# zhangzhousuper/Radish_PT

Measured on AMD Instinct MI355X. Metric: Mrays/s, higher is better.
Workload: dtype f32

## Files before the change

### radish_pt_amd/csrc/device/kernels_wave.h

```cpp
#pragma once
#include "kernels_pt.h"
#include "wg_trace.h"
#include "ray_cull.h"

namespace rd {

constexpr int kWfLitCap = 8192;
constexpr int kWfLitShadow = 0x40000000;
constexpr int kMaxWaveDepth = 32;

struct alignas(128) WaveCounter {
    int v;
    int pad[31];
};
#ifndef RD_WF_TICKET_SHARDS
#define RD_WF_TICKET_SHARDS 8
#endif
constexpr int kTicketShards = RD_WF_TICKET_SHARDS;
struct WaveCounters {
    WaveCounter rayCount[kMaxWaveDepth + 2];
    WaveCounter shadowCount[kMaxWaveDepth + 2];
    WaveCounter litCount[kMaxWaveDepth + 2];
    WaveCounter litShadowCount[kMaxWaveDepth + 2];
    WaveCounter traceHead[kMaxWaveDepth + 2];
    WaveCounter shadeHead[kMaxWaveDepth + 2][4];
    WaveCounter traceTicket[kMaxWaveDepth + 2][kTicketShards];
    WaveCounter shadeTicket[kMaxWaveDepth + 2][kTicketShards];
};

struct WaveWorkspace {
    float4 *ro[2];
    float4 *rd[2];
    float4 *thr[2];
    float4 *prevPos[2];
    float4 *accD;
    float4 *accI;
    float4 *nee[2];
    float4 *sht[2];
    uint2 *rng[2];
    int4 *hit;
    int *rayq[2];
    int *shadowq;
    int *litq[2];
    int litCap;
    int *treeOvf;
    int treeOvfDepth;
#ifdef RD_WF_STAMPS
    unsigned long long *stamps;
    int stampWaves;
    int stampStages;
#endif
    WaveCounters *ctr;
};

constexpr unsigned kWfNeeNone = 2u;
RD_DEV float wfNeeTag(int home, unsigned kind) { return __uint_as_float(((unsigned)home << 2) | kind); }
RD_DEV void wfAddNee(const WaveWorkspace &w, float4 n) {
    const unsigned tag = __float_as_uint(n.w), kind = tag & 3u;
    if (kind == kWfNeeNone) return;
    float4 *acc = (kind == 0u ? w.accD : w.accI) + (tag >> 2);
    const float4 a = *acc;
    *acc = make_float4(a.x + n.x, a.y + n.y, a.z + n.z, 0.f);
}

RD_DEV Ray wfSlotRay(const WaveWorkspace &w, int set, int p, bool shadow, float &limit) {
    if (shadow) {
        const float4 x = w.prevPos[set][p], y = w.sht[set][p];
        return shadowRay(mk3(x.x, x.y, x.z), mk3(y.x, y.y, y.z), limit);
    }
    const float4 o = w.ro[set][p], d = w.rd[set][p];
    limit = 3.402823466e+38f;
    return Ray{mk3(o.x, o.y, o.z), mk3(d.x, d.y, d.z)};
}

struct WaveSlotPath {
    const WaveWorkspace &w;
    const int rs, p;
    const int wr, q;
    int home;
    const bool delta;
    bool nullNee = false;
    RD_DEV v3 throughput() {
        const float4 t = w.thr[rs][p];
        home = __float_as_int(t.w);
        return mk3(t.x, t.y, t.z);
    }
// ... 335 lines not shown
                    if (busy && cur >= 0) {
                        pairStep<COUNT>(s.pairs, stk, lane, ovf, rs, tmax, ord, cur, sp, pending, ws);
                        busy = pending < 0 && (cur >= 0 || sp.sp > 0);
                    }
                } while (__popcll(__ballot(busy)) >= (minWalk > 1 ? minWalk : 1));
                alive = alive && (pending >= 0 || cur >= 0 || sp.sp > 0);
            }
        } else
        {
            bool walking = alive && pending < 0;
            const int nStart = __popcll(__ballot(walking));
#if RD_WF_COOP_LONE
            if (nStart == 1) {
                const int L = __ffsll((long long)__ballot(walking)) - 1;
                CoopResult cr = coopWalk(readlanePtr(nodes, L), readlaneI(node, L), end, readlaneRay(rs, L), readlaneF(tmax, L), RD_COOP_WINDOWS);
                if (int(threadIdx.x & 63u) == L) {
                    node = cr.node;
                    pending = cr.pending;
                    if (COUNT) ws.nodes += cr.visited;
                    alive = (node != end) || pending >= 0;
                }
            } else
#endif
            if (nStart > 0) {
                const int minWalk = (nStart * (RD_LEAF_DEN - RD_LEAF_NUM) + RD_LEAF_DEN - 1) / RD_LEAF_DEN;
                do {
                    if (walking) {
                        if (COUNT) ws.nodes++;
                        float4 lo = nodes[node].lo_prim;
                        float4 hi = nodes[node].hi_next;
                        float boundDist;
                        bool boundHit = aabbFast(lo, hi, rs, boundDist);
                        if (boundHit && boundDist < tmax) {
                            pending = __float_as_int(lo.w);
                            node++;
                        } else {
                            node = __float_as_int(hi.w);
                        }
                        walking = pending < 0 && node != END;
                        alive = (node != END) || pending >= 0;
                    }
                } while (__popcll(__ballot(walking)) >= (minWalk > 1 ? minWalk : 1));
            }
        }
        if (alive && pending >= 0) {
            TriVerts t = loadTri(s.tris, pending);
            float dist;
            v2 bary;
            if (COUNT) ws.tris++;
            bool hit = intersectTriangle(rs, t.a, t.b, t.c, bary, dist);
            if (hit && dist < tmax) {
                if (isShadow) {
                    occluded = true;
                    node = END;
                    cur = kPairNone;
                    sp = PairStack{0, 0};
                } else {
                    hitPrim = pending;
                    tmax = dist;
                    hitBary = bary;
                }
            }
            pending = -1;
            alive = PAIRS ? (cur >= 0 || sp.sp > 0) : (node != END);
        }
        const unsigned long long doneM = __ballot(!alive && p >= 0);
        if (doneM != 0ull && __popcll(doneM) * 64 >= (__popcll(doneM) + __popcll(__ballot(alive))) * RD_WF_FINISH_MIN)
        if (!alive && p >= 0) {
            if (isShadow) {
                if (!occluded) wfAddNee(w, w.nee[set][p]);
            } else {
                bool hit = hitPrim != -1;
                if (hit) nHits++;
                w.hit[p] = make_int4(hitPrim, __float_as_int(hit ? hitBary.x : 0.f), __float_as_int(hit ? hitBary.y : 0.f),
                                     hit ? int(s.primClass[hitPrim]) : 0);
            }
            p = -1;
        }
    }
    RD_WF_STAMP(2);
    if (COUNT) flushCounters(s.counters, nClosest, nAny, nHits, ws);
}

constexpr int kSortChunks = 16;
constexpr int kSortPacket = 64 * kSortChunks;
#ifndef RD_WF_SHADE_WAVES
#define RD_WF_SHADE_WAVES 1
#endif
#ifndef RD_WF_CULL_LAST
#define RD_WF_CULL_LAST 1
#endif
#ifndef RD_WF_SKIP_NULL_NEE
#define RD_WF_SKIP_NULL_NEE 1
#endif
__global__ __launch_bounds__(256, RD_WF_SHADE_WAVES) void k_wf_shade(DScene s, WaveWorkspace w, int k, int maxDepth, int sorted,
                                                                     const float4 *__restrict__ emitBox, int walkAll) {
    __shared__ int sSorted[4][kSortPacket];
    WaveCounters *c = w.ctr;
    const bool cullLast = RD_WF_CULL_LAST && !walkAll && k + 1 == maxDepth && !hasEnvMap(s);
    const bool skipNull = RD_WF_SKIP_NULL_NEE && !walkAll;
    float4 boxLo = make_float4(0.f, 0.f, 0.f, 0.f), boxHi = boxLo;
    if (cullLast) {
        boxLo = emitBox[0];
        boxHi = emitBox[1];
    }
    const int wg = workgroupTicket(c->shadeTicket[k]);
    const int lane = int(threadIdx.x & 63u);
    int *mySorted = sSorted[threadIdx.x >> 6];
    {
        const int q = 0;
        const int n = c->rayCount[k].v;
        const int *hitq = w.rayq[k & 1];
        int pendShadows = 0, pendRays = 0;
        int packet = kShadePacket;
        if (sorted) {
            const int perWave = n / (2 * gridWaves());
            packet = ((perWave + kShadePacket - 1) / kShadePacket) * kShadePacket;
            packet = packet < kShadePacket ? kShadePacket : (packet > kSortPacket ? kSortPacket : packet);
        }
        int packetEnd = 0;
        for (int base = logicalWave(wg) * packet, sub = 0, fresh = 1;;) {
            if (sub == packet) {
                base = wavePull(&c->shadeHead[k][q].v, packet);
                sub = 0;
                fresh = 1;
            }
            if (base + sub >= n) break;
            if (sorted && fresh) {
                fresh = 0;
                packetEnd = (n - base) < packet ? (n - base) : packet;
                int pp[kSortChunks], cls[kSortChunks];
#pragma unroll
                for (int j = 0; j < kSortChunks; j++) {
                    const int i = base + j * 64 + lane;
                    pp[j] = (j * 64 + lane < packetEnd) ? hitq[i] : -1;
                    if (pp[j] <= -2) pp[j] = -2 - pp[j];
                }
#pragma unroll
                for (int j = 0; j < kSortChunks; j++) {
                    cls[j] = (pp[j] >= 0) ? w.hit[pp[j]].w : 0;
                }
                int at = 0;
#pragma unroll
                for (int qq = 0; qq < 4; qq++) {
#pragma unroll
                    for (int j = 0; j < kSortChunks; j++) {
                        const bool in = (j * 64 + lane < packetEnd) && cls[j] == qq;
                        const unsigned long long m = __ballot(in);
                        if (in) mySorted[at + __popcll(m & laneMaskLt())] = pp[j];
                        at += __popcll(m);
                    }
                }
                __builtin_amdgcn_wave_barrier();
            }
            int item = base + sub + lane;
            const int subNow = sub;
            sub += 64;
            bool active = sorted ? (subNow + lane < packetEnd) : (item < n);
            bool emitShadow = false, emitRay = false, litShadow = false, litRay = false, rayFirst = false;
            int p = -1;
            const int q = base + subNow + lane;
            if (active) {
                p = sorted ? mySorted[subNow + lane] : hitq[item];
                if (p <= -2) p = -2 - p;
                active = p >= 0;
            }
// ... 89 lines not shown
```

### radish_pt_amd/csrc/radish_hip.hip

```cpp
#include "radish_hip.h"

#include <hip/hip_runtime.h>
#include <dlfcn.h>

#include <algorithm>
#include <cfloat>
#include <climits>
#include <cmath>
#include <cstdarg>
#include <cstdio>
#include <cstring>
#include <mutex>
#include <string>
#include <type_traits>
#include <utility>
#include <vector>

#include "device/kernels_pt.h"
#include "device/kernels_restir.h"
#include "device/kernels_wave.h"
#include "device/kernels_persist.h"
#include "device/kernels_walk.h"
#include "device/kernels_gbuffer.h"
#include "device/kernels_display.h"
// ... 482 lines not shown
            pend[c0 + nb] = pend[b] + 1;
            pend[c0 + (nb ^ 1)] = pend[b];
            if (pend[b] + 1 > depth) depth = pend[b] + 1;
        }
    }
    for (int box = 0; box < S; box++) {
        const int b = canon[box];
        const float *q = d->boundingBoxes + 6 * (size_t)box;
        tree[b].lo_prim = make_float4(q[0], q[1], q[2], asFloat(w3[b]));
        tree[b].hi_next = make_float4(q[3], q[4], q[5], asFloat(bits[b]));
    }
    pairs.assign((size_t)(S - 1) / 2 + 1, PairRec{});
    auto childW = [&](int b) { return w3[b] >= 0 ? w3[b] : ~((~w3[b] - 1) / 2); };
    for (int b = 0; b < S; b++) {
        if (w3[b] >= 0) continue;
        const int c0 = ~w3[b], q = (c0 - 1) / 2;
        const float4 l0 = tree[c0].lo_prim, h0 = tree[c0].hi_next, l1 = tree[c0 + 1].lo_prim, h1 = tree[c0 + 1].hi_next;
        pairs[q].lo0_w0 = make_float4(l0.x, l0.y, l0.z, asFloat(childW(c0)));
        pairs[q].hi0_bits = make_float4(h0.x, h0.y, h0.z, asFloat(bits[b]));
        pairs[q].lo1_w1 = make_float4(l1.x, l1.y, l1.z, asFloat(childW(c0 + 1)));
        pairs[q].hi1_pad = make_float4(h1.x, h1.y, h1.z, asFloat(0));
    }
    return true;
}

struct HostCamera {
    int32_t resx, resy;
    float position[3], rotation[3], view[3], up[3], right[3];
    float fov[2], pixelLength[2];
    float rotationMatInv[9];
    float viewProjection[16];
    float lensRadius, focalDist, tanFovY;
};
static_assert(sizeof(HostCamera) == 196, "Camera layout");

DCamera toDeviceCamera(const void *camera196) {
    HostCamera h;
    memcpy(&h, camera196, sizeof(h));
    DCamera d;
    d.resx = h.resx;
    d.resy = h.resy;
    d.position = {h.position[0], h.position[1], h.position[2]};
    d.view = {h.view[0], h.view[1], h.view[2]};
    d.up = {h.up[0], h.up[1], h.up[2]};
    d.right = {h.right[0], h.right[1], h.right[2]};
    d.rotationMatInv.c0 = {h.rotationMatInv[0], h.rotationMatInv[1], h.rotationMatInv[2]};
    d.rotationMatInv.c1 = {h.rotationMatInv[3], h.rotationMatInv[4], h.rotationMatInv[5]};
    d.rotationMatInv.c2 = {h.rotationMatInv[6], h.rotationMatInv[7], h.rotationMatInv[8]};
    d.lensRadius = h.lensRadius;
    d.focalDist = h.focalDist;
    d.tanFovY = tanf(h.fov[1] * 0.01745329251994329576923690768489f);
    return d;
}

PixelMap makePixelMap(const rdh_ctx *c) {
    PixelMap pm;
    pm.W = c->cam.resx;
    pm.H = c->cam.resy;
    pm.tile = c->tile;
    pm.tilesX = (pm.W + pm.tile - 1) / pm.tile;
    int tilesY = (pm.H + pm.tile - 1) / pm.tile;
    pm.numTiles = pm.tilesX * tilesY;
    pm.rank = c->rank;
    pm.world = c->world;
    pm.tilesPerRank = (pm.numTiles + pm.world - 1) / pm.world;
    pm.packed = (c->world > 1 || c->forcePacked) ? 1 : 0;
    int bpe = pm.tile / 8;
    pm.numBlocks = pm.tilesPerRank * bpe * bpe;
    return pm;
}

constexpr int kPairMinNodes = 0;
bool usePairs(const rdh_ctx *c, uint32_t flags) {
    if (!c->scene.ds.pairs || (flags & RDH_PT_NO_PAIRS)) return false;
    if (flags & RDH_PT_PAIRS) return true;
    if (c->pairMode >= 0) return c->pairMode != 0;
    return c->scene.ds.bvhSize >= kPairMinNodes;
}

bool usePackets(uint32_t flags) {
    static const int env = getenv("RADISH_PACKETS") ? atoi(getenv("RADISH_PACKETS")) : 1;
    return env != 0 && !(flags & RDH_PT_NO_PACKETS);
}

unsigned gridFor(const PixelMap &pm) {
    unsigned work = (unsigned)(pm.numBlocks + 3) / 4;
    return ((work + 7u) / 8u) * 8u;
}

unsigned gridBlocks(const PixelMap &pm) { return (((unsigned)pm.numBlocks + 7u) / 8u) * 8u; }

int settleTree(rdh_ctx *c) {
    if (!c->scene.treePending) return RDH_OK;
    HIP_TRY(c, hipEventSynchronize(c->evTree));
    c->scene.treePending = false;
    if (c->scene.treeRefit) {
        c->scene.treeRefit = false;
        if (!c->scene.ds.pairs) return RDH_OK;
        const int4 lo = c->hTreeHdr.as<int4>()[1], hi = c->hTreeHdr.as<int4>()[2];
        c->scene.ds.rootLo = make_float4(__builtin_bit_cast(float, lo.x), __builtin_bit_cast(float, lo.y), __builtin_bit_cast(float, lo.z), c->scene.ds.rootLo.w);
        c->scene.ds.rootHi = make_float4(__builtin_bit_cast(float, hi.x), __builtin_bit_cast(float, hi.y), __builtin_bit_cast(float, hi.z), c->scene.ds.rootHi.w);
        return RDH_OK;
    }
    const int4 *hdr = c->hTreeHdr.as<int4>(), h0 = hdr[0], lo = hdr[1], hi = hdr[2];
    if (h0.y != 0) {
        c->scene.haveScene = false;
        return fail(c, RDH_ERR_STATE, "device BVH build failed (error bits %d); the scene must be uploaded again", h0.y);
    }
    constexpr int kMaxPairDepth = 2048;
    const PairRec *pairs = c->scene.updPairs ? c->scene.updPairs : c->scene.ds.pairs;
    if (h0.x <= kMaxPairDepth) {
        c->scene.ds.pairs = pairs;
        c->scene.ds.treeDepth = h0.x;
        c->scene.ds.rootLo = make_float4(__builtin_bit_cast(float, lo.x), __builtin_bit_cast(float, lo.y), __builtin_bit_cast(float, lo.z),
                                   __builtin_bit_cast(float, lo.w));
        c->scene.ds.rootHi = make_float4(__builtin_bit_cast(float, hi.x), __builtin_bit_cast(float, hi.y), __builtin_bit_cast(float, hi.z),
                                   __builtin_bit_cast(float, hi.w));
    } else {
        c->scene.ds.pairs = nullptr;
        c->scene.ds.treeDepth = 0;
    }
    return RDH_OK;
}

int settleLights(rdh_ctx *c) {
    if (!c->scene.lightsPending) return RDH_OK;
    HIP_TRY(c, hipEventSynchronize(c->evLights));
    c->scene.lightsPending = false;
    c->scene.ds.sumLightPowerInv = c->hLightSums.as<float>()[1];
    return RDH_OK;
}

int requireReady(rdh_ctx *c) {
    if (!c) return RDH_ERR_ARGS;
    if (c->scene.haveScene) {
        int rc = settleTree(c);
        if (rc) return rc;
        if ((rc = settleLights(c))) return rc;
    }
    if (!c->scene.haveScene) return fail(c, RDH_ERR_NO_SCENE, "no scene uploaded (rdh_scene_upload)");
    if (!c->haveCamera) return fail(c, RDH_ERR_NO_SCENE, "no camera set (rdh_set_camera)");
    return RDH_OK;
}

constexpr size_t kProfilePairs = 8192;

long profBegin(rdh_ctx *c, uint32_t flags) {
    if (!(flags & RDH_PT_PROFILE) || c->profUsed >= kProfilePairs) return -1;
    if (c->profEvents.size() < 2 * (c->profUsed + 1)) {
        hipEvent_t a = nullptr, b = nullptr;
        if (newEvent(c, &a, true) || newEvent(c, &b, true)) return -1;
        c->profEvents.push_back(a);
        c->profEvents.push_back(b);
    }
    long i = (long)c->profUsed++;
    hipEventRecord(c->profEvents[2 * i], c->stream);
    return i;
}
void profEnd(rdh_ctx *c, long i) {
    if (i >= 0) hipEventRecord(c->profEvents[2 * i + 1], c->stream);
}

constexpr unsigned kPersistentGrid = 256u * 8u;

template <typename T>
int wfAlloc(rdh_ctx *c, T **out, size_t count) {
    void *p = nullptr;
    HIP_TRY(c, hipMalloc(&p, std::max<size_t>(count * sizeof(T), 16)));
    c->wfAllocs.push_back(p);
    *out = static_cast<T *>(p);
    return RDH_OK;
}

int wavefrontEnsureSlots(rdh_ctx *c, long long slots) {
    if (c->wfCapacity >= slots) return RDH_OK;
    for (void *p : c->wfAllocs) hipFree(p);
    c->wfAllocs.clear();
    c->wfCapacity = 0;
    const size_t n0 = (size_t)slots, n1 = (size_t)((slots / 64 + 1) / 2) * 64;
    for (int h = 0; h < kWfParts; h++) {
        WaveWorkspace &w = c->wf[h];
        const size_t n = h == 0 ? n0 : n1;
        int rc = RDH_OK;
        for (int set = 0; set < 2 && rc == RDH_OK; set++) {
            if ((rc = wfAlloc(c, &w.ro[set], n)) || (rc = wfAlloc(c, &w.rd[set], n)) || (rc = wfAlloc(c, &w.thr[set], n)) ||
                (rc = wfAlloc(c, &w.prevPos[set], n)) || (rc = wfAlloc(c, &w.nee[set], n)) || (rc = wfAlloc(c, &w.sht[set], n)) ||
                (rc = wfAlloc(c, &w.rng[set], n)))
                return rc;
        }
        if ((rc = wfAlloc(c, &w.accD, n)) || (rc = wfAlloc(c, &w.accI, n)) ||
            (rc = wfAlloc(c, &w.hit, n)) || (rc = wfAlloc(c, &w.rayq[0], n)) || (rc = wfAlloc(c, &w.rayq[1], n)) ||
            (rc = wfAlloc(c, &w.shadowq, n)) || (rc = wfAlloc(c, &w.ctr, 1)) || (rc = wfAlloc(c, &w.litq[0], (size_t)kWfLitCap)) ||
            (rc = wfAlloc(c, &w.litq[1], (size_t)kWfLitCap)))
            return rc;
        w.litCap = 0;
    }
    if (!c->evWfFork) {
        int rc;
        if ((rc = newEvent(c, &c->evWfFork)) || (rc = newEvent(c, &c->evWfJoin))) return rc;
        HIP_TRY(c, hipStreamCreateWithFlags(&c->wfStream, hipStreamNonBlocking));
        if ((rc = newEvent(c, &c->evWfJoin3))) return rc;
    }
    c->wfCapacity = slots;
    return RDH_OK;
}
int wavefrontEnsure(rdh_ctx *c, const PixelMap &pm, int samples) {
    return wavefrontEnsureSlots(c, (long long)pm.numBlocks * 64 * samples);
}

struct WfLaunch {
    bool count, sort, walkAll, tree;
    unsigned traceGrid, shadeGrid;
    int parts;
};
int wavefrontPrepare(rdh_ctx *c, int maxDepth, uint32_t flags, int parts, WfLaunch &L) {
    if (maxDepth > kMaxWaveDepth) return fail(c, RDH_ERR_ARGS, "maxDepth %d exceeds %d", maxDepth, kMaxWaveDepth);
    const bool count = (flags & RDH_PT_COUNT) != 0, sort = (flags & RDH_PT_SORT_MATERIAL) != 0;
    const bool walkAll = count || (flags & RDH_PT_WALK_ALL) != 0 || c->scene.lightListPartial;
    const bool tree = usePairs(c, flags);
    unsigned traceRes = 0, shadeRes = 0;
    int rq = RDH_OK;
    withBools([&](auto cnt, auto pr) { rq = residentGrid(c, k_wf_trace<cnt.value, pr.value>, 256, &traceRes); }, count, tree);
    if (rq || (rq = residentGrid(c, k_wf_shade, 256, &shadeRes))) return rq;
    if (tree && !count) {
        int cus = 0;
        if (int rc = cuCount(c, &cus)) return rc;
        traceRes = std::min(traceRes, (unsigned)cus * (unsigned)RD_WF_PAIR_MAX_WAVES);
    }
    const unsigned traceGrid = sharedGrid(c, std::min(traceRes, kPersistentGrid), kUnbounded);
    const unsigned shadeGrid = sharedGrid(c, std::min(shadeRes, kPersistentGrid), kUnbounded);
    const int ovfDepth = c->scene.ds.treeDepth + 1;
    const size_t ovfNeed = (size_t)traceGrid * 4 * 64 * (size_t)ovfDepth * 2;
    if (tree && parts > 1 && (size_t)parts * ovfNeed * sizeof(int) > kWfStripBudget) parts = 1;
    if (tree) {
        for (int h = 0; h < parts; h++) {
            if (int rc = grow(c, c->wfTreeOvf[h], ovfNeed, ovfNeed * sizeof(int), Busy::Device)) return rc;
            c->wf[h].treeOvf = c->wfTreeOvf[h].as<int>();
            c->wf[h].treeOvfDepth = ovfDepth;
        }
    }
#ifdef RD_WF_STAMPS
    {
        const size_t stamps = (size_t)(maxDepth + 1) * traceGrid * 4 * kWfStampKinds + (size_t)(maxDepth + 1);
        if (int rc = grow(c, c->wfStamps, stamps, stamps * sizeof(unsigned long long), Busy::Device)) return rc;
        HIP_TRY(c, hipMemsetAsync(c->wfStamps.p, 0, stamps * sizeof(unsigned long long), c->stream));
        for (int h = 0; h < kWfParts; h++) {
            c->wf[h].stamps = h == 0 ? c->wfStamps.as<unsigned long long>() : nullptr;
            c->wf[h].stampWaves = (int)(traceGrid * 4);
            c->wf[h].stampStages = maxDepth + 1;
        }
        c->wfStampStages = maxDepth + 1;
        c->wfStampWaves = (int)(traceGrid * 4);
    }
#endif
    if (!c->scene.emitBox)
        if (int rc = sceneAlloc(c, &c->scene.emitBox, 2 * sizeof(float4))) return rc;
    if (RD_WF_CULL_LAST && !walkAll && maxDepth >= 1 && c->scene.ds.envTex < 0) {
        hipLaunchKernelGGL(k_emitter_bounds, dim3(1), dim3(256), 0, c->stream, c->scene.ds.tris, (const int *)c->scene.dLightPrims,
                           c->scene.numLights, c->scene.ds.bvhSize > 0 ? c->scene.ds.nodes[0] : nullptr, c->scene.emitBox);
        HIP_TRY(c, hipGetLastError());
    }
    c->wfLastStages = maxDepth + 1;
    c->wfLastParts = parts;
    for (int h = 0; h < parts; h++) {
        const unsigned waves = traceGrid * 4u;
        c->wf[h].litCap = (int)(waves * 64u < (unsigned)kWfLitCap ? waves * 64u : (unsigned)kWfLitCap);
        if (flags & RDH_PT_WF_SMALL_LISTS) c->wf[h].litCap = 4;
    }
    L = WfLaunch{count, sort, walkAll, tree, traceGrid, shadeGrid, parts};
    return RDH_OK;
}

void keepHip(rdh_ctx *c, int &rc, hipError_t e, const char *what) {
    if (e != hipSuccess && rc == RDH_OK) rc = fail(c, (int)e, "HIP error (%s): %s: %s", __FILE__, what, hipGetErrorString(e));
}

void wavefrontStages(rdh_ctx *c, const WfLaunch &L, int maxDepth, uint32_t flags, int &rc) {
    hipStream_t sts[kWfParts] = {c->stream, c->sideStream, c->wfStream};
    for (int k = 0; k <= maxDepth && rc == RDH_OK; k++) {
        for (int h = 0; h < L.parts; h++) {
            hipStream_t st = sts[h];
            WaveWorkspace &w = c->wf[h];
            long pe = (h == 0 && L.parts == 1) ? profBegin(c, flags) : -1;
            withBools([&](auto cnt, auto pr) {
                hipLaunchKernelGGL((k_wf_trace<cnt.value, pr.value>), dim3(L.traceGrid), dim3(256), 0, st, c->scene.ds, w, k);
            }, L.count, L.tree);
            profEnd(c, pe);
            hipLaunchKernelGGL(k_wf_shade, dim3(L.shadeGrid), dim3(256), 0, st, c->scene.ds, w, k, maxDepth, L.sort ? 1 : 0,
                               (const float4 *)c->scene.emitBox, L.walkAll ? 1 : 0);
        }
        keepHip(c, rc, hipGetLastError(), "wavefront stage launch");
    }
}

int wavefrontPathTrace(rdh_ctx *c, const PixelMap &pm, float *d_direct, float *d_indirect, int iter, int looper, int samples,
                       int maxDepth, uint32_t flags) {
    static const int partsEnv = getenv("RADISH_WF_PARTS") ? atoi(getenv("RADISH_WF_PARTS")) : kWfPartsDefault;
    WfLaunch L;
    if (int rq = wavefrontPrepare(c, maxDepth, flags, ((flags & RDH_PT_WF_SUBFRAMES) && pm.numBlocks >= 2048) ?
                                  (partsEnv >= 1 && partsEnv <= kWfParts ? partsEnv : kWfPartsDefault) : 1, L))
        return rq;
    const int parts = L.parts;
    hipStream_t sts[kWfParts] = {c->stream, c->sideStream, c->wfStream};
    const long pf = parts >= 2 ? profBegin(c, flags) : -1;
    if (parts >= 2) {
        HIP_TRY(c, hipEventRecord(c->evWfFork, c->stream));
        for (int h = 1; h < parts; h++) HIP_TRY(c, hipStreamWaitEvent(sts[h], c->evWfFork, 0));
    }
    int rc = RDH_OK;
    auto keep = [&](hipError_t e, const char *what) { keepHip(c, rc, e, what); };
    for (int h = 0; h < parts; h++) {
        hipStream_t st = sts[h];
        WaveWorkspace &w = c->wf[h];
        const unsigned nLocal = (unsigned)(pm.numBlocks - h + parts - 1) / (unsigned)parts;
        const unsigned gridBlk = (((nLocal * (unsigned)samples + 3u) / 4u + 7u) / 8u) * 8u;
        keep(hipMemsetAsync(w.ctr, 0, sizeof(WaveCounters), st), "hipMemsetAsync(wavefront counters)");
        hipLaunchKernelGGL(k_wf_raygen, dim3(gridBlk), dim3(256), 0, st, c->scene.ds, c->cam, pm, w, looper, samples, h, parts);
    }
    wavefrontStages(c, L, maxDepth, flags, rc);
    for (int h = 0; h < parts && rc == RDH_OK; h++) {
        hipStream_t st = sts[h];
        const unsigned nLocal = (unsigned)(pm.numBlocks - h + parts - 1) / (unsigned)parts;
        const unsigned gridBlk = (((nLocal + 3u) / 4u + 7u) / 8u) * 8u;
        hipLaunchKernelGGL(k_wf_finish, dim3(gridBlk), dim3(256), 0, st, pm, c->wf[h], iter, samples, d_direct, d_indirect, h, parts);
    }
    keep(hipGetLastError(), "k_wf_finish");
    if (parts >= 2) {
        hipError_t e1 = hipEventRecord(c->evWfJoin, c->sideStream);
        hipError_t e2 = hipStreamWaitEvent(c->stream, c->evWfJoin, 0);
        hipError_t e3 = hipEventRecord(c->evWfJoin3, c->wfStream);
        hipError_t e4 = hipStreamWaitEvent(c->stream, c->evWfJoin3, 0);
        if (e1 != hipSuccess || e2 != hipSuccess || e3 != hipSuccess || e4 != hipSuccess) {
            hipStreamSynchronize(c->sideStream);
            hipStreamSynchronize(c->wfStream);
            keep(e1 != hipSuccess ? e1 : (e2 != hipSuccess ? e2 : (e3 != hipSuccess ? e3 : e4)), "wavefront join");
        }
    }
    profEnd(c, pf);
    return rc;
}

int ensureStackOverflow(rdh_ctx *c, unsigned resident) {
    const size_t ints = (size_t)resident * 64 * (size_t)(c->scene.ds.treeDepth + 1) * 2;
    return grow(c, c->treeOvf, ints, ints * sizeof(int), Busy::Device);
}

uint32_t resolveStructure(const rdh_ctx *c, const PixelMap &pm, uint32_t flags) {
    if (!(flags & RDH_PT_AUTO)) return flags;
    flags &= ~(RDH_PT_AUTO | RDH_PT_WAVEFRONT | RDH_PT_SORT_MATERIAL | RDH_PT_WF_SUBFRAMES | RDH_PT_PERSISTENT);
    const bool wavefront = c->scene.ds.bvhSize >= 100000 && pm.numBlocks >= 12000;
    return flags | (wavefront ? (RDH_PT_WAVEFRONT | RDH_PT_SORT_MATERIAL | RDH_PT_WF_SUBFRAMES) : RDH_PT_PERSISTENT);
}

int packetBudget(uint32_t flags) { return (flags & RDH_PT_WF_SMALL_LISTS) ? 4 : kPacketBudget; }

int launchWalk(rdh_ctx *c, const float *d_rays, long long n, int4 *d_hits, int *d_occ, bool count, const int *deferCount = nullptr,
               const int *deferList = nullptr, int slotList = 0, bool pairs = false, bool packets = false, int budget = kPacketBudget) {
    const bool any = d_occ != nullptr, defer = deferCount != nullptr;
    packets = packets && !any && n > 0 && (n + 255) / 256 <= 0x7fffffffll;
    if (pairs && !c->scene.ds.pairs) return fail(c, RDH_ERR_UNSUPPORTED, "RDH_PT_PAIRS: the uploaded node arrays are not six orderings of one binary tree, or that tree is more than 2 048 levels deep");
    unsigned resGrid = 0;
    int rc = RDH_OK;
    withBools([&](auto a) {
        rc = pairs ? residentGrid(c, k_walk_pair<false, a.value>, 64, &resGrid) : residentGrid(c, k_walk_persistent<false, a.value>, 64, &resGrid);
    }, any);
    if (rc) return rc;
    const unsigned grid = sharedGrid(c, resGrid, (unsigned long long)((n + 63) / 64));
    const int ovfDepth = c->scene.ds.treeDepth + 1;
    if (pairs && !packets && (rc = ensureStackOverflow(c, resGrid))) return rc;
    int2 *const ovf = c->treeOvf.as<int2>();
    if (!packets) HIP_TRY(c, hipMemsetAsync(c->dPersist, 0, offsetof(PersistCounters, deferred), c->stream));
    if (defer) {
        if ((rc = forkLiteral(c))) return rc;
        withBools([&](auto cnt, auto a) {
            hipLaunchKernelGGL((k_trace_wg_list<cnt.value, a.value>), dim3(kWalkDeferCap), dim3(kWgTraceThreads), 0, c->litStream, c->scene.ds, d_rays, deferList, deferCount, d_hits, d_occ);
        }, count, any);
    }
    if (packets) {
        const unsigned pgrid = (unsigned)((n + 255) / 256);
        withBools([&](auto cnt, auto def) {
            hipLaunchKernelGGL((k_walk_packet<cnt.value, def.value>), dim3(pgrid), dim3(256), 0, c->stream, c->scene.ds, d_rays, n, d_hits, deferCount, slotList, budget);
        }, count, defer);
    } else {
        withBools([&](auto cnt, auto a, auto def) {
            if (pairs)
                hipLaunchKernelGGL((k_walk_pair<cnt.value, a.value, def.value>), dim3(grid), dim3(64), 0, c->stream, c->scene.ds, d_rays, n, d_hits, d_occ,
                                   c->dPersist, ovf, ovfDepth, deferCount, slotList);
            else
                hipLaunchKernelGGL((k_walk_persistent<cnt.value, a.value, def.value>), dim3(grid), dim3(64), 0, c->stream, c->scene.ds, d_rays, n, d_hits, d_occ,
                                   c->dPersist, deferCount, slotList);
        }, count, any, defer);
    }
    if (defer) joinLiteral(c);
    HIP_TRY(c, hipGetLastError());
    return RDH_OK;
}

RestirSplit splitLayout(Carver &k, size_t slots) {
    RestirSplit sp;
    sp.st = k.take<float4>(slots * 48);
    sp.hits = k.take<int4>(slots * 16);
    sp.rays = k.take<float>(slots * 24);
    sp.segs = k.take<float>(slots * 24);
    sp.rawResv = k.take<float>(slots * 36);
    sp.occ = k.take<int>(slots * 4);
    sp.deferCount = k.take<int>(16 + 2 * sizeof(int) * kRestirDeferCap);
    sp.deferList = sp.deferCount + 4;
    return sp;
}

void timeBegin(rdh_ctx *c) {
    hipEventRecord(c->evStart, c->stream);
}
int timeEnd(rdh_ctx *c, const char *what) {
    hipEventRecord(c->evStop, c->stream);
    c->timed = true;
    hipError_t e = hipGetLastError();
    if (e != hipSuccess) return fail(c, (int)e, "HIP error: %s: %s", what, hipGetErrorString(e));
    return RDH_OK;
}

}

extern "C" {

int rdh_create(rdh_ctx **out, int device) {
    if (!out) return RDH_ERR_ARGS;
    *out = nullptr;
    int n = 0;
    if (hipGetDeviceCount(&n) != hipSuccess || n <= 0 || device < 0 || device >= n) return RDH_ERR_NO_DEVICE;
    if (hipSetDevice(device) != hipSuccess) return RDH_ERR_NO_DEVICE;
    rdh_ctx *c = new rdh_ctx;
    c->device = device;
    if (hipStreamCreateWithFlags(&c->ownStream, hipStreamNonBlocking) != hipSuccess ||
        newEvent(c, &c->evStart, true) || newEvent(c, &c->evStop, true) ||
        hipStreamCreateWithFlags(&c->sideStream, hipStreamNonBlocking) != hipSuccess ||
        newEvent(c, &c->evFork) || newEvent(c, &c->evJoin) || newEvent(c, &c->evFrame) || newEvent(c, &c->evSched[0]) ||
// ... 409 lines not shown
            return fail(c, RDH_ERR_ARGS, "rdh_path_trace_samples: %d samples per pass of %lld path slots each: a pass holds fewer than 2^30 "
                        "slots and at most %zu MiB of them (%lld samples here)", perPass, frameSlots, kWfSampleBudget >> 20, cap);
        perPass = (int)cap;
    }
    HIP_TRY(c, hipSetDevice(c->device));
    if ((rc = wavefrontEnsure(c, pm, perPass))) return rc;
    timeBegin(c);
    for (int s = 0; s < numSamples; s += perPass) {
        const int b = std::min(perPass, numSamples - s);
        if ((rc = wavefrontPathTrace(c, pm, d_direct, d_indirect, iter + s, (looper + s) % kSobolRows, b, maxDepth, flags))) return rc;
    }
    return timeEnd(c, "pathTrace (wavefront)");
}

namespace {
struct AdaptScratch {
    AdaptiveHead *head;
    AdaptiveStats *stats;
    int *wgTotals;
};
static_assert(sizeof(rdh_adaptive_stats) == sizeof(AdaptiveStats) && sizeof(AdaptiveStats) == 16, "rdh_adaptive_stats layout");
int adaptiveScratch(rdh_ctx *c, size_t groups, AdaptScratch &a) {
    if (int rc = growCarved(c, c->adaptScan, groups, Busy::Stream, [&](Carver &k) {
            a.head = k.take<AdaptiveHead>(sizeof(AdaptiveHead));
            a.stats = k.take<AdaptiveStats>(sizeof(AdaptiveStats));
            a.wgTotals = k.take<int>(groups * sizeof(int));
        }))
        return rc;
    return grow(c, c->hAdapt, 1, std::max(sizeof(AdaptiveHead), sizeof(AdaptiveStats)), Busy::Nothing);
}
}

int rdh_path_trace_adaptive(rdh_ctx *c, float *d_direct, float *d_indirect, int32_t *d_count, const int32_t *d_request, float *d_moments,
                            int looper, int maxDepth, uint32_t flags, int64_t *samplesTraced) {
    int rc = requireReady(c);
    if (rc) return rc;
    if (!d_direct || !d_indirect || !d_count || !d_request || looper < 0 || looper >= kSobolRows || maxDepth < 0)
        return fail(c, RDH_ERR_ARGS, "rdh_path_trace_adaptive: bad arguments");
    if (4 + 7 * maxDepth > 200) return fail(c, RDH_ERR_ARGS, "maxDepth %d needs more than 200 Sobol dimensions", maxDepth);
    if (!(flags & RDH_PT_WAVEFRONT) || (flags & (RDH_PT_PERSISTENT | RDH_PT_AUTO)))
        return fail(c, RDH_ERR_UNSUPPORTED, "rdh_path_trace_adaptive: only the wavefront pipeline traces a slot list (RDH_PT_WAVEFRONT, "
                    "without RDH_PT_PERSISTENT or RDH_PT_AUTO)");
    const PixelMap pm = makePixelMap(c);
    if (pm.world > 1 || pm.packed)
        return fail(c, RDH_ERR_UNSUPPORTED, "rdh_path_trace_adaptive: the planes are in frame layout; a tile partition (world %d) is not supported", pm.world);
    if ((long long)pm.numBlocks * 64 > kAdaptiveMaxWork)
        return fail(c, RDH_ERR_ARGS, "rdh_path_trace_adaptive: %lld pixel slots of the frame, a slot's owner names fewer than %lld",
                    (long long)pm.numBlocks * 64, kAdaptiveMaxWork);
    HIP_TRY(c, hipSetDevice(c->device));
    if (samplesTraced) *samplesTraced = 0;
    const unsigned groups = ((unsigned)pm.numBlocks + 3u) / 4u;
    AdaptScratch a;
    if ((rc = adaptiveScratch(c, groups, a))) return rc;
    HIP_TRY(c, hipMemsetAsync(a.head, 0, sizeof(AdaptiveHead), c->stream));
    hipLaunchKernelGGL(k_ad_count, dim3(groups), dim3(256), 0, c->stream, pm, (const int *)d_count, (const int *)d_request, a.wgTotals, a.head);
    hipLaunchKernelGGL(k_ad_scan, dim3(1), dim3(256), 0, c->stream, a.wgTotals, (int)groups, a.head);
    HIP_TRY(c, hipGetLastError());
    AdaptiveHead *const head = c->hAdapt.as<AdaptiveHead>();
    HIP_TRY(c, hipMemcpyAsync(head, a.head, sizeof(AdaptiveHead), hipMemcpyDeviceToHost, c->stream));
    HIP_TRY(c, hipStreamSynchronize(c->stream));
    if (head->err)
        return fail(c, RDH_ERR_ARGS, "rdh_path_trace_adaptive: a request outside 0..%d, or a requested pixel's count negative or beyond "
                    "int32 with its request; nothing was traced", kAdaptiveMaxRequest);
    const long long T = head->total;
    if (T == 0) return RDH_OK;
    const long long padded = (T + 63) & ~63ll;
    const long long cap = std::min(kWfMaxSlots - 1, (long long)(kWfSampleBudget / kWfSlotBytes));
    if (padded > cap)
        return fail(c, RDH_ERR_ARGS, "rdh_path_trace_adaptive: %lld requested samples: a pass holds fewer than 2^30 path slots and at most "
                    "%zu MiB of them (%lld slots); lower the step", T, kWfSampleBudget >> 20, cap);
    if ((rc = grow(c, c->adaptOwners, (size_t)padded, (size_t)padded * sizeof(int), Busy::Stream))) return rc;
    if ((rc = wavefrontEnsureSlots(c, padded))) return rc;
    WfLaunch L;
    if ((rc = wavefrontPrepare(c, maxDepth, flags, 1, L))) return rc;
    timeBegin(c);
    WaveWorkspace &w = c->wf[0];
    int *const owner = c->adaptOwners.as<int>();
    hipLaunchKernelGGL(k_ad_scatter, dim3(groups), dim3(256), 0, c->stream, pm, (const int *)d_request, (const int *)a.wgTotals, (int)T, owner);
    keepHip(c, rc, hipMemsetAsync(w.ctr, 0, sizeof(WaveCounters), c->stream), "hipMemsetAsync(wavefront counters)");
    const unsigned genGrid = ((((unsigned)(padded / 64) + 3u) / 4u + 7u) / 8u) * 8u;
    hipLaunchKernelGGL(k_ad_raygen, dim3(genGrid), dim3(256), 0, c->stream, c->scene.ds, c->cam, pm, w, looper, (const int *)d_count,
                       (const int *)owner, (int)T);
    keepHip(c, rc, hipGetLastError(), "k_ad_raygen");
    wavefrontStages(c, L, maxDepth, flags, rc);
    if (rc == RDH_OK) {
        hipLaunchKernelGGL(k_ad_finish, dim3((unsigned)((T + 255) / 256)), dim3(256), 0, c->stream, pm, w, (const int *)owner, (int)T,
                           d_count, (const int *)d_request, d_direct, d_indirect, d_moments);
        keepHip(c, rc, hipGetLastError(), "k_ad_finish");
    }
    if (rc) return rc;
    if (samplesTraced) *samplesTraced = T;
    return timeEnd(c, "pathTrace (adaptive)");
}

int rdh_adaptive_plan(rdh_ctx *c, const int32_t *d_count, const float *d_moments, int32_t *d_request, int minSamples, int maxSamples,
                      int step, float threshold, rdh_adaptive_stats *out) {
    if (!c) return RDH_ERR_ARGS;
    if (!c->haveCamera) return fail(c, RDH_ERR_NO_SCENE, "no camera set (rdh_set_camera)");
    if (!d_count || !d_moments || !d_request || step < 1 || step > kAdaptiveMaxRequest || minSamples < 0 || maxSamples < minSamples ||
        !(threshold >= 0.f && threshold <= FLT_MAX))
        return fail(c, RDH_ERR_ARGS, "rdh_adaptive_plan: bad arguments (step 1..%d, 0 <= minSamples <= maxSamples, a finite threshold >= 0)",
                    kAdaptiveMaxRequest);
    const PixelMap pm = makePixelMap(c);
    if (pm.world > 1 || pm.packed)
        return fail(c, RDH_ERR_UNSUPPORTED, "rdh_adaptive_plan: the planes are in frame layout; a tile partition (world %d) is not supported", pm.world);
    HIP_TRY(c, hipSetDevice(c->device));
    const unsigned groups = ((unsigned)pm.numBlocks + 3u) / 4u;
    AdaptScratch a;
    if (int rc = adaptiveScratch(c, groups, a)) return rc;
    HIP_TRY(c, hipMemsetAsync(a.stats, 0, sizeof(AdaptiveStats), c->stream));
    hipLaunchKernelGGL(k_ad_plan, dim3(groups), dim3(256), 0, c->stream, pm, (const int *)d_count, d_moments, (int *)d_request, minSamples,
                       maxSamples, step, threshold, a.stats);
    HIP_TRY(c, hipGetLastError());
    if (out) {
        HIP_TRY(c, hipMemcpyAsync(c->hAdapt.p, a.stats, sizeof(AdaptiveStats), hipMemcpyDeviceToHost, c->stream));
        HIP_TRY(c, hipStreamSynchronize(c->stream));
        memcpy(out, c->hAdapt.p, sizeof(AdaptiveStats));
    }
    return RDH_OK;
}

int rdh_path_trace_direct(rdh_ctx *c, float *d_direct, int iter, int looper, uint32_t flags) {
    int rc = requireReady(c);
    if (rc) return rc;
    if (!d_direct || iter < 0 || looper < 0 || looper >= 10000) return fail(c, RDH_ERR_ARGS, "rdh_path_trace_direct: bad arguments");
    HIP_TRY(c, hipSetDevice(c->device));
    PixelMap pm = makePixelMap(c);
    timeBegin(c);
    withBools([&](auto cnt) {
        hipLaunchKernelGGL(k_path_trace_direct<cnt.value>, dim3(gridBlocks(pm)), dim3(64), 0, c->stream, c->scene.ds, c->cam, pm, looper,
                           iter, d_direct);
    }, (flags & RDH_PT_COUNT) != 0);
    return timeEnd(c, "pathTraceDirect");
}

static int enqueueGBuffer(rdh_ctx *c, const rdh_gbuffer *gb, uint32_t flags);

int rdh_gbuffer_render(rdh_ctx *c, const rdh_gbuffer *gb, uint32_t flags) {
    int rc = requireReady(c);
    if (rc) return rc;
    if ((rc = enqueueGBuffer(c, gb, flags))) return rc;
    c->scene.movedSinceRender = false;
    return RDH_OK;
}

static int enqueueGBuffer(rdh_ctx *c, const rdh_gbuffer *gb, uint32_t flags) {
    int rc;
    if (!gb || !gb->albedo || !gb->motion || (gb->frameIdx & ~1)) return fail(c, RDH_ERR_ARGS, "rdh_gbuffer_render: bad G-buffer");
    for (int k = 0; k < 2; k++)
        if (!gb->normal[k] || !gb->depth[k] || !gb->primId[k]) return fail(c, RDH_ERR_ARGS, "rdh_gbuffer_render: null plane");
    if (gb->width != c->cam.resx || gb->height != c->cam.resy)
        return fail(c, RDH_ERR_ARGS, "G-buffer %dx%d does not match camera %dx%d", gb->width, gb->height, c->cam.resx, c->cam.resy);
    HIP_TRY(c, hipSetDevice(c->device));
    if ((rc = waitExchanges(c, true, false))) return rc;
    PixelMap pm = makePixelMap(c);
    pm.packed = 0;
    if (c->world > 1 && !(flags & RDH_PT_PARTITION_GBUFFER)) {
        pm.rank = 0;
        pm.world = 1;
        pm.tilesPerRank = pm.numTiles;
        pm.packed = 0;
        pm.numBlocks = pm.numTiles * (pm.tile / 8) * (pm.tile / 8);
    }
    DCamera last = toDeviceCamera(gb->lastCam);
    GBufPtrs p{gb->albedo, gb->normal[gb->frameIdx], gb->motion, gb->depth[gb->frameIdx], gb->primId[gb->frameIdx],
               gb->width, gb->height, c->scene.movedSinceRender ? c->scene.prevTris : nullptr};
// ... 2248 lines not shown
```

Measured before the change: 3393.

## Trace primary wavefront rays with coherent packet walker instead of generic trace

For depth 0 of the wavefront path tracer, a new k_wf_trace_primary kernel runs the set-aside rays cooperatively per workgroup, then walks the coherent primary rays in 64-ray packets with the existing walkPacket traversal. Primary rays from the camera are coherent, so packet traversal can share node fetches and cut divergence compared with the per-ray persistent trace kernel. The cost is a one-workgroup-per-64-ray-group launch shape instead of a persistent grid, plus a different occupancy bound, and it is only used when packets are enabled and the BVH is non-empty.

```diff
diff --git a/radish_pt_amd/csrc/device/kernels_wave.h b/radish_pt_amd/csrc/device/kernels_wave.h
--- a/radish_pt_amd/csrc/device/kernels_wave.h
+++ b/radish_pt_amd/csrc/device/kernels_wave.h
@@ -2,6 +2,7 @@
 #include "kernels_pt.h"
 #include "wg_trace.h"
 #include "ray_cull.h"
+#include "kernels_walk.h"
 
 namespace rd {
 
@@ -503,6 +504,58 @@
     if (COUNT) flushCounters(s.counters, nClosest, nAny, nHits, ws);
 }
 
+struct WfSlotWork {
+    const WaveWorkspace &w;
+    int p;
+
+    RD_DEV bool find(long long chunk, int slot) {
+        const int e = w.rayq[0][chunk * 64 + slot];
+        p = e <= -2 ? -2 - e : e;
+        return e != -1;
+    }
+    RD_DEV Ray ray(float &tmax) const { return wfSlotRay(w, 0, p, false, tmax); }
+    RD_DEV void store(const DScene &s, const RaySlab &, int hitPrim, v2 hitBary, float, bool) const {
+        const bool hit = hitPrim != -1;
+        w.hit[p] = make_int4(hitPrim, __float_as_int(hit ? hitBary.x : 0.f), __float_as_int(hit ? hitBary.y : 0.f),
+                             hit ? int(s.primClass[hitPrim]) : 0);
+    }
+};
+#ifndef RD_WF_PRIMARY_WAVES
+#define RD_WF_PRIMARY_WAVES 1
+#endif
+template <bool COUNT>
+__global__ __launch_bounds__(256, COUNT ? 1 : RD_WF_PRIMARY_WAVES) void k_wf_trace_primary(DScene s, WaveWorkspace w, int nGroups, int budget) {
+    __shared__ WgTraceSharedT<256> wgsh;
+    const int nLit = w.ctr->litCount[0].v < w.litCap ? w.ctr->litCount[0].v : w.litCap;
+    WalkStats ws{0, 0};
+    unsigned nClosest = 0, nHits = 0;
+    for (int it = int(blockIdx.x); it < nLit; it += int(gridDim.x)) {
+        const int pp = w.litq[0][it];
+        float lim;
+        const Ray ray = wfSlotRay(w, 0, pp, false, lim);
+        const RaySlab urs = makeRaySlab(ray);
+        if (!raySetAside(urs.cls) || s.bvhSize == 0) continue;
+        const CoopTrace ct = wgTraceWhole<false, 256>(s, s.nodes[getMTBVHId(-ray.d)], urs, lim, wgsh);
+        if (threadIdx.x == 0) {
+            nClosest++;
+            const bool hit = ct.hitPrim != -1;
+            if (hit) nHits++;
+            w.hit[pp] = make_int4(ct.hitPrim, __float_as_int(hit ? ct.bary.x : 0.f), __float_as_int(hit ? ct.bary.y : 0.f),
+                                  hit ? int(s.primClass[ct.hitPrim]) : 0);
+            if (COUNT) {
+                ws.nodes += ct.nodes;
+                ws.tris += ct.tris;
+            }
+        }
+    }
+    if (COUNT && threadIdx.x < 64u) flushCounters(s.counters, nClosest, 0u, nHits, ws);
+    const int group = int(blockIdx.x) * 4 + int(threadIdx.x >> 6);
+    if (group >= nGroups) return;
+    const bool listed = w.rayq[0][(size_t)group * 64 + (threadIdx.x & 63u)] <= -2;
+    WfSlotWork work{w, -1};
+    walkPacket<COUNT, true>(s, group, listed, budget, work);
+}
+
 constexpr int kSortChunks = 16;
 constexpr int kSortPacket = 64 * kSortChunks;
 #ifndef RD_WF_SHADE_WAVES
diff --git a/radish_pt_amd/csrc/radish_hip.hip b/radish_pt_amd/csrc/radish_hip.hip
--- a/radish_pt_amd/csrc/radish_hip.hip
+++ b/radish_pt_amd/csrc/radish_hip.hip
@@ -588,6 +588,7 @@
     static const int env = getenv("RADISH_PACKETS") ? atoi(getenv("RADISH_PACKETS")) : 1;
     return env != 0 && !(flags & RDH_PT_NO_PACKETS);
 }
+int packetBudget(uint32_t flags) { return (flags & RDH_PT_WF_SMALL_LISTS) ? 4 : kPacketBudget; }
 
 unsigned gridFor(const PixelMap &pm) {
     unsigned work = (unsigned)(pm.numBlocks + 3) / 4;
@@ -718,6 +719,8 @@
     bool count, sort, walkAll, tree;
     unsigned traceGrid, shadeGrid;
     int parts;
+    unsigned primaryGroups[kWfParts] = {0, 0, 0};
+    int primaryBudget = 0;
 };
 int wavefrontPrepare(rdh_ctx *c, int maxDepth, uint32_t flags, int parts, WfLaunch &L) {
     if (maxDepth > kMaxWaveDepth) return fail(c, RDH_ERR_ARGS, "maxDepth %d exceeds %d", maxDepth, kMaxWaveDepth);
@@ -774,6 +777,7 @@
         if (flags & RDH_PT_WF_SMALL_LISTS) c->wf[h].litCap = 4;
     }
     L = WfLaunch{count, sort, walkAll, tree, traceGrid, shadeGrid, parts};
+    L.primaryBudget = (usePackets(flags) && c->scene.ds.bvhSize > 0) ? packetBudget(flags) : 0;
     return RDH_OK;
 }
 
@@ -788,9 +792,16 @@
             hipStream_t st = sts[h];
             WaveWorkspace &w = c->wf[h];
             long pe = (h == 0 && L.parts == 1) ? profBegin(c, flags) : -1;
-            withBools([&](auto cnt, auto pr) {
-                hipLaunchKernelGGL((k_wf_trace<cnt.value, pr.value>), dim3(L.traceGrid), dim3(256), 0, st, c->scene.ds, w, k);
-            }, L.count, L.tree);
+            if (k == 0 && L.primaryBudget > 0 && L.primaryGroups[h] > 0) {
+                withBools([&](auto cnt) {
+                    hipLaunchKernelGGL((k_wf_trace_primary<cnt.value>), dim3((L.primaryGroups[h] + 3u) / 4u), dim3(256), 0, st, c->scene.ds, w,
+                                       (int)L.primaryGroups[h], L.primaryBudget);
+                }, L.count);
+            } else {
+                withBools([&](auto cnt, auto pr) {
+                    hipLaunchKernelGGL((k_wf_trace<cnt.value, pr.value>), dim3(L.traceGrid), dim3(256), 0, st, c->scene.ds, w, k);
+                }, L.count, L.tree);
+            }
             profEnd(c, pe);
             hipLaunchKernelGGL(k_wf_shade, dim3(L.shadeGrid), dim3(256), 0, st, c->scene.ds, w, k, maxDepth, L.sort ? 1 : 0,
                                (const float4 *)c->scene.emitBox, L.walkAll ? 1 : 0);
@@ -820,6 +831,7 @@
         WaveWorkspace &w = c->wf[h];
         const unsigned nLocal = (unsigned)(pm.numBlocks - h + parts - 1) / (unsigned)parts;
         const unsigned gridBlk = (((nLocal * (unsigned)samples + 3u) / 4u + 7u) / 8u) * 8u;
+        L.primaryGroups[h] = nLocal * (unsigned)samples;
         keep(hipMemsetAsync(w.ctr, 0, sizeof(WaveCounters), st), "hipMemsetAsync(wavefront counters)");
         hipLaunchKernelGGL(k_wf_raygen, dim3(gridBlk), dim3(256), 0, st, c->scene.ds, c->cam, pm, w, looper, samples, h, parts);
     }
@@ -857,8 +869,6 @@
     const bool wavefront = c->scene.ds.bvhSize >= 100000 && pm.numBlocks >= 12000;
     return flags | (wavefront ? (RDH_PT_WAVEFRONT | RDH_PT_SORT_MATERIAL | RDH_PT_WF_SUBFRAMES) : RDH_PT_PERSISTENT);
 }
-
-int packetBudget(uint32_t flags) { return (flags & RDH_PT_WF_SMALL_LISTS) ? 4 : kPacketBudget; }
 
 int launchWalk(rdh_ctx *c, const float *d_rays, long long n, int4 *d_hits, int *d_occ, bool count, const int *deferCount = nullptr,
                const int *deferList = nullptr, int slotList = 0, bool pairs = false, bool packets = false, int budget = kPacketBudget) {
@@ -1434,6 +1444,7 @@
     hipLaunchKernelGGL(k_ad_raygen, dim3(genGrid), dim3(256), 0, c->stream, c->scene.ds, c->cam, pm, w, looper, (const int *)d_count,
                        (const int *)owner, (int)T);
     keepHip(c, rc, hipGetLastError(), "k_ad_raygen");
+    L.primaryGroups[0] = (unsigned)(padded / 64);
     wavefrontStages(c, L, maxDepth, flags, rc);
     if (rc == RDH_OK) {
         hipLaunchKernelGGL(k_ad_finish, dim3((unsigned)((T + 255) / 256)), dim3(256), 0, c->stream, pm, w, (const int *)owner, (int)T,
```

New measurement: 3492 (median of 6 runs). +2.9%, better.
